# rodrigo-paganini/kalman-vae

Hardware: AMD Instinct MI355X
Metric: sequences/sec (ELBO training step, 32x32xT bouncing-ball) (higher is better)
Workload: dtype f32; 1 GPU; BASELINE configs[1] (configs[2] per-GPU shard): bouncing-ball 32x32, T=50, batch=256/GPU, dynamics=lstm K=3, z=4, u=4, a=2, full train step (fwd incl. sigmoid(x_logits) + loss incl. active-unit stats + bwd + clip + Adam); both the GPU leg and the cpu_baseline leg do this work; preset=c2, global_batch=256, seq_len=50, parallelism=dp1, capture=hipgraph, loss_finite=True, dist_backend=none

## Files before the change

### include/kvae_lgssm.h

```cpp
#ifndef KVAE_LGSSM_H
#define KVAE_LGSSM_H

#include <stdint.h>

#ifdef __cplusplus
extern "C" {
#endif

#define KVAE_MAX_DIM 16
#define KVAE_ABI_VERSION 11

typedef enum {
  KVAE_OK = 0,
  KVAE_ERR_DIMS = 1,
  KVAE_ERR_NULL = 2,
  KVAE_ERR_LAUNCH = 3,
  KVAE_ERR_ARG = 4
} kvae_status;

typedef struct {
  const float *ptr;
  int64_t sb, st;
} kvae_stack;

typedef struct {
  int32_t B, T, n, m, p;
  kvae_stack A;
  kvae_stack Bm;
  kvae_stack C;
  kvae_stack Q;
  const float *R;
  const float *mu0;
  int64_t mu0_sb;
// ... 125 lines not shown


int kvae_bce_frames_fwd(const float *logits, const float *x, float *frame_ll, int64_t frames, int32_t pixels, void *stream);
int kvae_bce_frames_bwd(const float *logits, const float *x, const float *g_frame, float *g_logits, int64_t frames,
                        int32_t pixels, void *stream);


#define KVAE_DEC_HEAD_SCRATCH_FLOATS 2304
int kvae_dec_head_fwd(const float *in, const float *W, const float *bias, float *logits, float *w_scratch, int64_t N,
                      int32_t Cin, int32_t side, void *stream);
int kvae_dec_head_bwd(const float *in, const float *W, const float *g_logits, float *g_in, float *w_partials,
                      float *b_partials, float *w_scratch, int64_t N, int32_t Cin, int32_t side, void *stream);
int kvae_enc_stem_fwd(const float *x, const float *W, const float *bias, float *out, uint32_t *relu_bits, int64_t N, int32_t Cout,
                      int32_t side, void *stream);
int kvae_enc_stem_bwd(const float *x, const float *out, const uint32_t *relu_bits, const float *g_out, float *w_partials,
                      float *b_partials, int64_t N, int32_t Cout, int32_t side, void *stream);
int64_t kvae_conv_edge_partial_rows(int64_t N);

int kvae_enc_mid_fwd(const float *in, const float *W, const float *bias, float *out, int64_t N, int32_t C, int32_t side,
                     void *stream);
int kvae_enc_mid_bwd(const float *in, const float *W, const float *out, const float *g_out, float *g_in,
                     float *w_partials, float *b_partials, int64_t N, int32_t C, int32_t side, void *stream);
int64_t kvae_enc_mid_partial_rows(int64_t N, int32_t side);

int kvae_dec_up_fwd(const float *x, const float *W, const float *bias, float *out, int64_t N, int32_t Cin, int32_t side,
                    void *stream);
int kvae_dec_up_bwd(const float *x, const float *W, const float *out, const float *g_out, float *g_x, float *w_partials,
                    float *b_partials, int64_t N, int32_t Cin, int32_t side, void *stream);
int64_t kvae_dec_up_partial_rows(int64_t N, int32_t side);
int32_t kvae_dec_up_set_workgroups(int32_t n);


int kvae_enc_head_fwd(const float *feat, const float *Wmu, const float *bmu, const float *Wvar, const float *bvar,
                      const float *eps, float *mu, float *var, float *a, int64_t N, int32_t F, int32_t A,
                      float noise_emission, void *stream);
int kvae_enc_head_bwd(const float *feat, const float *Wmu, const float *Wvar, const float *var, const float *eps,
                      const float *g_a, const float *g_mu, const float *g_var, float *g_feat, float *w_partials,
                      float *b_partials, int64_t N, int32_t F, int32_t A, float noise_emission, void *stream);
int kvae_dec_fc_fwd(const float *a, const float *W, const float *b, float *h, int64_t N, int32_t F, int32_t A, void *stream);
int kvae_dec_fc_bwd(const float *g_h, const float *a, const float *W, float *g_a, float *w_partials, float *b_partials,
                    int64_t N, int32_t F, int32_t A, void *stream);
int64_t kvae_head_partial_rows(void);
int kvae_latent_reg_fwd(const float *a, const float *mu, const float *var, float *reg, int64_t N, int32_t A, void *stream);
int kvae_latent_reg_bwd(const float *a, const float *mu, const float *var, const float *g, float *g_a, float *g_mu,
                        float *g_var, int64_t N, int32_t A, void *stream);

// ... 49 lines not shown
```

### kalman-vae_amd/csrc/kvae_vae.hip

```cpp
#include <hip/hip_runtime.h>

#include <stdint.h>
#include <stdio.h>
#include <stdlib.h>
#include <string.h>

#include "../../include/kvae_lgssm.h"

namespace kvae {}
using namespace kvae;

extern "C" int kvae_launch_status(const char *what);
static int launch_status(const char *what) { return kvae_launch_status(what); }

#include "vae_epilogue.h"

__device__ __forceinline__ void colsum_v4_body(const float *__restrict__ partials, float *__restrict__ out, int64_t rows, int64_t cols,
                                               unsigned block) {
  __shared__ float4 red[8][64];
  const int lane = threadIdx.x & 63, wv = threadIdx.x >> 6;
  const int64_t c = ((int64_t)block * 64 + lane) * 4;
  float4 s0 = make_float4(0.f, 0.f, 0.f, 0.f), s1 = s0, s2 = s0, s3 = s0;
  if (c < cols) {
    const float *p = partials + c;
// ... 399 lines not shown
  if (N < 1 || (N + 256 * 8) * EM_C * side * side * 4 >= EM_MAX_BYTES) return KVAE_ERR_ARG;
  if (C != EM_C || (side != 16 && side != 8)) return KVAE_ERR_DIMS;
  const dim3 grid((unsigned)enc_mid_grid(N, side));
  if (side == 16) k_enc_mid_fwd<16><<<grid, dim3(256), 0, (hipStream_t)stream>>>(in, W, bias, out, N);
  else k_enc_mid_fwd<8><<<grid, dim3(256), 0, (hipStream_t)stream>>>(in, W, bias, out, N);
  return launch_status("k_enc_mid_fwd");
}
int kvae_enc_mid_bwd(const float *in, const float *W, const float *out, const float *g_out, float *g_in,
                     float *w_partials, float *b_partials, int64_t N, int32_t C, int32_t side, void *stream) {
  if (!in || !W || !out || !g_out || !w_partials || !b_partials) return KVAE_ERR_NULL;
  if (N < 1 || (N + 256 * 8) * EM_C * side * side * 4 >= EM_MAX_BYTES) return KVAE_ERR_ARG;
  if (C != EM_C || (side != 16 && side != 8)) return KVAE_ERR_DIMS;
  const dim3 grid((unsigned)enc_mid_grid(N, side));
  if (g_in) {
    if (side == 16) k_enc_mid_bwd_data<16><<<grid, dim3(256), 0, (hipStream_t)stream>>>(W, out, g_out, g_in, N);
    else k_enc_mid_bwd_data<8><<<grid, dim3(256), 0, (hipStream_t)stream>>>(W, out, g_out, g_in, N);
    const int rc = launch_status("k_enc_mid_bwd_data");
    if (rc) return rc;
  }
  if (side == 16) k_enc_mid_wrw<16><<<grid, dim3(256), 0, (hipStream_t)stream>>>(in, out, g_out, w_partials, b_partials, N);
  else k_enc_mid_wrw<8><<<grid, dim3(256), 0, (hipStream_t)stream>>>(in, out, g_out, w_partials, b_partials, N);
  return launch_status("k_enc_mid_wrw");
}
}

#include "vae_conv_up_wino.h"
static bool dec_up_wino() {
  static const int env = getenv("KVAE_WINO") ? atoi(getenv("KVAE_WINO")) : 1;
  return env != 0;
}
static int g_dec_up_wgs = 0;
static inline int64_t dec_up_cap() {
  static const int env = getenv("KVAE_UP_WGS") ? atoi(getenv("KVAE_UP_WGS")) : 0;
  const int v = env >= 1 && env <= 256 ? env : __atomic_load_n(&g_dec_up_wgs, __ATOMIC_RELAXED);
  return v >= 1 && v <= 256 ? v : 256;
}
static inline int64_t dec_up_grid(int64_t N, int32_t side) {
  const int64_t fpi = side == 8 ? 2 : 8, iters = (N + fpi - 1) / fpi, cap = dec_up_cap();
  return iters < cap ? (iters < 1 ? 1 : iters) : cap;
}
extern "C" {
int64_t kvae_dec_up_partial_rows(int64_t N, int32_t side) { return dec_up_grid(N, side); }
int32_t kvae_dec_up_set_workgroups(int32_t n) {
  const int32_t prev = (int32_t)dec_up_cap();
  __atomic_store_n(&g_dec_up_wgs, n >= 1 && n <= 256 ? n : 0, __ATOMIC_RELAXED);
  return prev;
// ... 117 lines not shown
```

### kalman-vae_amd/csrc/vae_epilogue.h

```cpp
#pragma once
#include <stdint.h>

#include "lgssm_vm.h"

namespace kvae {

struct EpiShape { int64_t N; int C, H, W, r; };

KV_DEV int64_t epi_src(const EpiShape &s, int64_t o, int *ch) {
  const int OW = s.W * s.r, OH = s.H * s.r;
  const int ow = (int)(o % OW);
  const int64_t t1 = o / OW;
  const int oh = (int)(t1 % OH);
  const int64_t t2 = t1 / OH;
  const int c = (int)(t2 % s.C);
  const int64_t n = t2 / s.C;
  const int cc = c * s.r * s.r + (oh % s.r) * s.r + (ow % s.r);
  *ch = cc;
  return ((n * (s.C * s.r * s.r) + cc) * s.H + oh / s.r) * s.W + ow / s.r;
}

KV_DEV void epi_fwd_elem(const EpiShape &s, const float *in, const float *bias, float *out, int64_t o, int relu) {
  int ch;
  const int64_t i = epi_src(s, o, &ch);
  float v = in[i] + bias[ch];
  if (relu) v = v > 0.f ? v : 0.f;
  out[o] = v;
}

KV_DEV void epi_bwd_elem(const EpiShape &s, const float *g_out, const float *out, float *g_in, int64_t o, int relu) {
  int ch;
  const int64_t i = epi_src(s, o, &ch);
  float g = g_out[o];
  if (relu && !(out[o] > 0.f)) g = 0.f;
  g_in[i] = g;
}

}
```

### kalman-vae_amd/kvae/_native.py

```python
import ctypes as C
import os
from pathlib import Path

import torch

_HERE = Path(__file__).resolve().parent
LIB_PATH = _HERE / "lib" / "libkvae_lgssm.so"

KVAE_MAX_DIM = 16
KVAE_MAX_K = 16
LSTM_MAX_H, LSTM_MAX_I = 52, 16
ABI_VERSION = 11

_STATUS = {1: "KVAE_ERR_DIMS (n, m, p must be in [1,16]; B, T >= 1)", 2: "KVAE_ERR_NULL", 3: "KVAE_ERR_LAUNCH",
           4: "KVAE_ERR_ARG"}


class Stack(C.Structure):
    _fields_ = [("ptr", C.c_void_p), ("sb", C.c_int64), ("st", C.c_int64)]


class Problem(C.Structure):
    _fields_ = [("B", C.c_int32), ("T", C.c_int32), ("n", C.c_int32), ("m", C.c_int32), ("p", C.c_int32),
                ("A", Stack), ("Bm", Stack), ("C", Stack), ("Q", Stack),
                ("R", C.c_void_p), ("mu0", C.c_void_p), ("mu0_sb", C.c_int64),
                ("Sigma0", C.c_void_p), ("Sigma0_sb", C.c_int64),
                ("Y", C.c_void_p), ("U", C.c_void_p), ("mask", C.c_void_p)]


class States(C.Structure):
    _fields_ = [(k, C.c_void_p) for k in ("mus_filt", "Sigmas_filt", "mus_pred", "Sigmas_pred",
                                          "mus_smooth", "Sigmas_smooth", "aux")]


class WgradProblem(C.Structure):
    _fields_ = [("d", C.c_void_p), ("h", C.c_void_p), ("x", C.c_void_p), ("g_wh", C.c_void_p), ("g_wx", C.c_void_p),
                ("g_b", C.c_void_p), ("d_stride", C.c_int64), ("h_stride", C.c_int64), ("x_stride", C.c_int64), ("N", C.c_int64),
                ("R", C.c_int32), ("H", C.c_int32), ("I", C.c_int32), ("bias", C.c_int32), ("T", C.c_int32), ("shift", C.c_int32)]


class GenProblem(C.Structure):
    _fields_ = ([(k, C.c_int32) for k in ("B", "S", "H", "n", "m", "p", "K", "kind", "hidden")]
                + [(k, C.c_void_p) for k in ("A", "Bm", "C", "LQ", "LR", "mu", "L0", "U", "w_ih", "w_hh", "b_ih", "b_hh",
                                             "head_w", "head_b", "h0", "c0", "y0", "P", "s0", "eps0", "eps_z", "eps_a",
                                             "gumbel", "a_out", "z_out", "w_out")])


class InputGrads(C.Structure):
    _fields_ = [("gA", Stack), ("gB", Stack), ("gC", Stack), ("gQ", Stack),
                ("gY", C.c_void_p), ("gU", C.c_void_p), ("g_mu0", C.c_void_p), ("g_Sigma0", C.c_void_p)]


SYMBOLS = ("kvae_lgssm_filter_alpha_lstm", "kvae_lgssm_alpha_lstm_bwd", "kvae_lgssm_filter_fwd", "kvae_lgssm_rts_fwd", "kvae_lgssm_smooth_fwd", "kvae_lgssm_smooth_bwd",
           "kvae_lgssm_elbo", "kvae_mix_fwd", "kvae_mix_bwd", "kvae_mix_bwd_partials", "kvae_lstm_fwd",
           "kvae_lstm_bwd", "kvae_bias_shuffle_act_fwd", "kvae_bias_shuffle_act_bwd", "kvae_bias_partial_rows", "kvae_colsum", "kvae_colsum2", "kvae_clip_adam", "kvae_regime_fwd", "kvae_regime_bwd", "kvae_bigru_fwd", "kvae_bigru_bwd", "kvae_bce_frames_fwd", "kvae_bce_frames_bwd",
           "kvae_dec_head_fwd", "kvae_dec_head_bwd", "kvae_enc_stem_fwd", "kvae_enc_stem_bwd", "kvae_conv_edge_partial_rows",
           "kvae_enc_mid_fwd", "kvae_enc_mid_bwd", "kvae_enc_mid_partial_rows",
           "kvae_dec_up_fwd", "kvae_dec_up_bwd", "kvae_dec_up_partial_rows", "kvae_dec_up_set_workgroups",
           "kvae_enc_head_fwd", "kvae_enc_head_bwd", "kvae_dec_fc_fwd", "kvae_dec_fc_bwd", "kvae_head_partial_rows",
           "kvae_latent_reg_fwd", "kvae_latent_reg_bwd", "kvae_loss_head_fwd", "kvae_loss_head_bwd",
           "kvae_lgssm_emission_means", "kvae_lgssm_generate", "kvae_rnn_wgrad", "kvae_rnn_wgrad_ws_floats", "kvae_linear_fwd", "kvae_linear_bwd_input",
           "kvae_abi_version",
           "kvae_last_error", "kvae_build_info")


class LgssmLib:

    def __init__(self, path):
        self.path = str(path)
        self.dll = C.CDLL(self.path)
        missing = [s for s in SYMBOLS if not hasattr(self.dll, s)]
        if missing:
            raise OSError(f"{self.path} does not export {missing}")
        d = self.dll
        P, S, G, vp = C.POINTER(Problem), C.POINTER(States), C.POINTER(InputGrads), C.c_void_p
        for name in ("kvae_lgssm_filter_fwd", "kvae_lgssm_rts_fwd", "kvae_lgssm_smooth_fwd"):
            getattr(d, name).argtypes = [P, S, vp]
            getattr(d, name).restype = C.c_int
        d.kvae_lgssm_filter_alpha_lstm.argtypes = [P, S] + [vp] * 9 + [C.c_int32, C.c_int32] + [vp] * 7
        d.kvae_lgssm_filter_alpha_lstm.restype = C.c_int
# ... 24 lines not shown
        d.kvae_regime_bwd.argtypes = [vp] * 10 + [C.c_int32] * 3 + [C.c_float, vp, vp]
        d.kvae_regime_bwd.restype = C.c_int
        d.kvae_bigru_fwd.argtypes = [vp] * 7 + [C.c_int32] * 4 + [vp]
        d.kvae_bigru_fwd.restype = C.c_int
        d.kvae_bigru_bwd.argtypes = [vp] * 8 + [C.c_int32] * 4 + [vp]
        d.kvae_bigru_bwd.restype = C.c_int
        d.kvae_bce_frames_fwd.argtypes = [vp, vp, vp, C.c_int64, C.c_int32, vp]
        d.kvae_bce_frames_fwd.restype = C.c_int
        d.kvae_bce_frames_bwd.argtypes = [vp, vp, vp, vp, C.c_int64, C.c_int32, vp]
        d.kvae_bce_frames_bwd.restype = C.c_int
        d.kvae_dec_head_fwd.argtypes = [vp, vp, vp, vp, vp, C.c_int64, C.c_int32, C.c_int32, vp]
        d.kvae_dec_head_fwd.restype = C.c_int
        d.kvae_dec_head_bwd.argtypes = [vp] * 7 + [C.c_int64, C.c_int32, C.c_int32, vp]
        d.kvae_dec_head_bwd.restype = C.c_int
        d.kvae_enc_stem_fwd.argtypes = [vp, vp, vp, vp, vp, C.c_int64, C.c_int32, C.c_int32, vp]
        d.kvae_enc_stem_fwd.restype = C.c_int
        d.kvae_enc_stem_bwd.argtypes = [vp] * 6 + [C.c_int64, C.c_int32, C.c_int32, vp]
        d.kvae_enc_stem_bwd.restype = C.c_int
        d.kvae_enc_mid_fwd.argtypes = [vp, vp, vp, vp, C.c_int64, C.c_int32, C.c_int32, vp]
        d.kvae_enc_mid_fwd.restype = C.c_int
        d.kvae_enc_mid_bwd.argtypes = [vp] * 7 + [C.c_int64, C.c_int32, C.c_int32, vp]
        d.kvae_enc_mid_bwd.restype = C.c_int
        d.kvae_enc_mid_partial_rows.argtypes = [C.c_int64, C.c_int32]
        d.kvae_dec_up_fwd.argtypes = [vp, vp, vp, vp, C.c_int64, C.c_int32, C.c_int32, vp]
        d.kvae_dec_up_fwd.restype = C.c_int
        d.kvae_dec_up_bwd.argtypes = [vp] * 7 + [C.c_int64, C.c_int32, C.c_int32, vp]
        d.kvae_dec_up_bwd.restype = C.c_int
        d.kvae_dec_up_partial_rows.argtypes = [C.c_int64, C.c_int32]
        d.kvae_enc_head_fwd.argtypes = [vp] * 9 + [C.c_int64, C.c_int32, C.c_int32, C.c_float, vp]
        d.kvae_enc_head_fwd.restype = C.c_int
        d.kvae_enc_head_bwd.argtypes = [vp] * 11 + [C.c_int64, C.c_int32, C.c_int32, C.c_float, vp]
        d.kvae_enc_head_bwd.restype = C.c_int
        d.kvae_dec_fc_fwd.argtypes = [vp] * 4 + [C.c_int64, C.c_int32, C.c_int32, vp]
        d.kvae_dec_fc_fwd.restype = C.c_int
        d.kvae_dec_fc_bwd.argtypes = [vp] * 6 + [C.c_int64, C.c_int32, C.c_int32, vp]
        d.kvae_dec_fc_bwd.restype = C.c_int
        d.kvae_head_partial_rows.argtypes = []
        d.kvae_head_partial_rows.restype = C.c_int64
        d.kvae_latent_reg_fwd.argtypes = [vp] * 4 + [C.c_int64, C.c_int32, vp]
        d.kvae_latent_reg_fwd.restype = C.c_int
        d.kvae_latent_reg_bwd.argtypes = [vp] * 7 + [C.c_int64, C.c_int32, vp]
        d.kvae_latent_reg_bwd.restype = C.c_int
        d.kvae_loss_head_fwd.argtypes = [vp] * 5 + [C.c_float] * 3 + [vp, vp, vp, C.c_int64, vp]
        d.kvae_loss_head_fwd.restype = C.c_int
        d.kvae_loss_head_bwd.argtypes = [vp, vp, vp, vp, vp, vp, C.c_int64, vp]
        d.kvae_loss_head_bwd.restype = C.c_int
# ... 153 lines not shown
```

### kalman-vae_amd/kvae/vae/fused.py

```python
import torch

from .. import _native as N


colsum = N.colsum
colsum_pair = N.colsum_pair


def _chunks(n, size):
    return [(a, min(a + size, n)) for a in range(0, n, size)]


def _acc(total, part):
    return part if total is None else total + part


class BiasShuffleAct(torch.autograd.Function):

    @staticmethod
    def forward(ctx, x, bias, r, relu):
        x = x.contiguous()
        bias = bias.contiguous()
        Nb, Crr, H, W = x.shape
        C = Crr // (r * r)
# ... 120 lines not shown
            lib.check(N.timed(f"enc_mid_fwd_s{s}", x, lambda: lib.dll.kvae_enc_mid_fwd(
                N.ptr(x[a:b]), N.ptr(weight), N.ptr(bias), N.ptr(out[a:b]), b - a, Cc, s, N.stream_for(x))), "kvae_enc_mid_fwd")
        ctx.save_for_backward(x, weight, out)
        return out

    @staticmethod
    def backward(ctx, g):
        x, weight, out = ctx.saved_tensors
        g = g.contiguous()
        Nb, Cc, s, _ = x.shape
        lib = N.lib_for(x)
        g_x = torch.empty_like(x) if ctx.needs_input_grad[0] else None
        gw = gb = None
        for a, b in _chunks(Nb, EncoderMid.CHUNK):
            rows = lib.dll.kvae_enc_mid_partial_rows(b - a, s)
            wp = torch.empty(rows, weight.numel(), device=x.device, dtype=torch.float32)
            bp = torch.empty(rows, Cc, device=x.device, dtype=torch.float32)
            lib.check(lib.dll.kvae_enc_mid_bwd(N.ptr(x[a:b]), N.ptr(weight), N.ptr(out[a:b]), N.ptr(g[a:b]),
                                               N.ptr(g_x[a:b]) if g_x is not None else None, N.ptr(wp), N.ptr(bp), b - a, Cc, s,
                                               N.stream_for(x)), "kvae_enc_mid_bwd")
            cw, cb = colsum_pair(wp, bp)
            gw, gb = _acc(gw, cw), _acc(gb, cb)
        return g_x, gw.view_as(weight), gb


class DecoderUp(torch.autograd.Function):

    CHUNK = 16384

    @staticmethod
    def supported(x, conv):
        return (x.dim() == 4 and x.shape[1] == 32 and x.shape[2] == x.shape[3] and x.shape[2] in (8, 4)
                and tuple(conv.weight.shape) == (128, 32, 3, 3) and conv.stride == (1, 1) and conv.padding == (1, 1)
                and conv.dilation == (1, 1) and conv.groups == 1 and conv.bias is not None)

    @staticmethod
    def forward(ctx, x, weight, bias):
        x, weight, bias = x.contiguous(), weight.contiguous(), bias.contiguous()
        Nb, Cin, s, _ = x.shape
        out = torch.empty(Nb, 32, 2 * s, 2 * s, device=x.device, dtype=torch.float32)
        lib = N.lib_for(x)
        for a, b in _chunks(Nb, DecoderUp.CHUNK):
            lib.check(N.timed(f"dec_up_fwd_s{s}", x, lambda: lib.dll.kvae_dec_up_fwd(
                N.ptr(x[a:b]), N.ptr(weight), N.ptr(bias), N.ptr(out[a:b]), b - a, Cin, s, N.stream_for(x))), "kvae_dec_up_fwd")
        ctx.save_for_backward(x, weight, out)
        return out
# ... 185 lines not shown
```

### kalman-vae_amd/kvae/vae/vae.py

```python
import os
from typing import Tuple

import torch
import torch.nn as nn

from kvae import _native
from kvae.utils.config import KVAEConfig
from kvae.vae.fused import DecoderFc, DecoderHead, DecoderUp, EncoderHead, EncoderMid, EncoderStem, conv_block


def _conv_out(size, k, s, p):
    return (size + 2 * p - k) // s + 1


class Encoder(nn.Module):

    def __init__(self, config: KVAEConfig):
        super().__init__()
        self.config = config
        blocks, c_in, side = [], config.img_channels, config.img_size
        for c_out in config.encoder_channels:
            blocks += [nn.Conv2d(c_in, c_out, config.encoder_kernel_size, config.encoder_stride,
                                 config.encoder_padding), nn.ReLU()]
            side = _conv_out(side, config.encoder_kernel_size, config.encoder_stride, config.encoder_padding)
            c_in = c_out
        self.conv_layers = nn.Sequential(*blocks)
        self.flat_size = c_in * side * side
        self.fc_mu = nn.Linear(self.flat_size, config.a_dim)
        self.fc_var = nn.Sequential(nn.Linear(self.flat_size, config.a_dim), nn.Sigmoid())

    def features(self, x: torch.Tensor) -> torch.Tensor:
        if _native.fused_ok(x) and x.dtype == torch.float32:
            h = x
            for i, layer in enumerate(self.conv_layers):
                if isinstance(layer, nn.Conv2d):
                    if i == 0 and EncoderStem.supported(h, layer):
                        h = EncoderStem.apply(h, layer.weight, layer.bias)
                    elif EncoderMid.supported(h, layer):
                        h = EncoderMid.apply(h, layer.weight, layer.bias)
                    else:
                        h = conv_block(h, layer, r=1, relu=True)
            return h.flatten(1)
        return self.conv_layers(x).flatten(1)

    def heads(self, feat: torch.Tensor, eps=None):
        if _native.fused_ok(feat) and feat.dtype == torch.float32 and EncoderHead.supported(feat, self.fc_mu, self.fc_var[0]):
            return EncoderHead.apply(feat, self.fc_mu.weight, self.fc_mu.bias, self.fc_var[0].weight, self.fc_var[0].bias,
                                     eps, self.config.noise_emission)
        mu, var = self.fc_mu(feat), self.config.noise_emission * self.fc_var(feat)
        return (mu if eps is None else mu + eps * torch.sqrt(var + 1e-6)), mu, var

    def forward(self, x: torch.Tensor) -> Tuple[torch.Tensor, torch.Tensor]:
        _, mu, var = self.heads(self.features(x))
        return mu, var


class Decoder(nn.Module):
# ... 80 lines not shown
```

Before: 95460 sequences/s.

## Fuse encoder stem and mid conv layers into single kernels

Adds fused kernels that compute the first encoder conv (1->32, stride 2) together with the second conv (32->32, 16x16->8x8). The stem output stays in registers and LDS, interleaved with the MFMA work of the mid conv, so the intermediate activation is never written to or read back from global memory. Only packed ReLU bitmasks are stored. The backward pass recomputes stem activations from x to produce weight gradients for both layers in two kernels. This saves an activation round-trip and several launches, at the cost of very complex hand-scheduled kernels and recomputation work. The path is enabled by default through an env var and only applies when the batch fits in one chunk.

```diff
diff --git a/include/kvae_lgssm.h b/include/kvae_lgssm.h
--- a/include/kvae_lgssm.h
+++ b/include/kvae_lgssm.h
@@ -8,7 +8,7 @@
 #endif
 
 #define KVAE_MAX_DIM 16
-#define KVAE_ABI_VERSION 11
+#define KVAE_ABI_VERSION 12
 
 typedef enum {
   KVAE_OK = 0,
@@ -180,6 +180,13 @@
 int kvae_enc_mid_bwd(const float *in, const float *W, const float *out, const float *g_out, float *g_in,
                      float *w_partials, float *b_partials, int64_t N, int32_t C, int32_t side, void *stream);
 int64_t kvae_enc_mid_partial_rows(int64_t N, int32_t side);
+
+int kvae_enc_stem_mid_fwd(const float *x, const float *W0, const float *b0, const float *W1, const float *b1, float *out,
+                          uint32_t *relu_bits, int64_t N, void *stream);
+int kvae_enc_stem_mid_bwd(const float *x, const float *W0, const float *b0, const float *W1, const uint32_t *relu_bits,
+                          const float *out, const float *g_out, float *w0_partials, float *b0_partials, float *w1_partials,
+                          float *b1_partials, int64_t N, void *stream);
+int64_t kvae_enc_stem_mid_partial_rows(int64_t N);
 
 int kvae_dec_up_fwd(const float *x, const float *W, const float *bias, float *out, int64_t N, int32_t Cin, int32_t side,
                     void *stream);
diff --git a/kalman-vae_amd/csrc/kvae_vae.hip b/kalman-vae_amd/csrc/kvae_vae.hip
--- a/kalman-vae_amd/csrc/kvae_vae.hip
+++ b/kalman-vae_amd/csrc/kvae_vae.hip
@@ -445,6 +445,29 @@
   else k_enc_mid_wrw<8><<<grid, dim3(256), 0, (hipStream_t)stream>>>(in, out, g_out, w_partials, b_partials, N);
   return launch_status("k_enc_mid_wrw");
 }
+
+int64_t kvae_enc_stem_mid_partial_rows(int64_t N) { return enc_mid_grid(N, 16); }
+int kvae_enc_stem_mid_fwd(const float *x, const float *W0, const float *b0, const float *W1, const float *b1, float *out,
+                          uint32_t *relu_bits, int64_t N, void *stream) {
+  if (!x || !W0 || !b0 || !W1 || !b1 || !out || !relu_bits) return KVAE_ERR_NULL;
+  if (N < 1 || (N + 256 * 8) * EM_C * 16 * 16 * 4 >= EM_MAX_BYTES) return KVAE_ERR_ARG;
+  k_enc_stem_mid_fwd<<<dim3((unsigned)enc_mid_grid(N, 16)), dim3(256), 0, (hipStream_t)stream>>>(x, W0, b0, W1, b1, out, relu_bits, N);
+  return launch_status("k_enc_stem_mid_fwd");
+}
+int kvae_enc_stem_mid_bwd(const float *x, const float *W0, const float *b0, const float *W1, const uint32_t *relu_bits,
+                          const float *out, const float *g_out, float *w0_partials, float *b0_partials, float *w1_partials,
+                          float *b1_partials, int64_t N, void *stream) {
+  if (!x || !W0 || !b0 || !W1 || !relu_bits || !out || !g_out || !w0_partials || !b0_partials || !w1_partials || !b1_partials)
+    return KVAE_ERR_NULL;
+  if (N < 1 || (N + 256 * 8) * EM_C * 16 * 16 * 4 >= EM_MAX_BYTES) return KVAE_ERR_ARG;
+  const dim3 grid((unsigned)enc_mid_grid(N, 16));
+  k_enc_stem_mid_bwd<<<grid, dim3(256), 0, (hipStream_t)stream>>>(x, W1, relu_bits, out, g_out, w0_partials, b0_partials, N,
+                                                                  kvae_conv_edge_partial_rows(N));
+  const int rc = launch_status("k_enc_stem_mid_bwd");
+  if (rc) return rc;
+  k_enc_stem_mid_wrw<<<grid, dim3(256), 0, (hipStream_t)stream>>>(x, W0, b0, out, g_out, w1_partials, b1_partials, N);
+  return launch_status("k_enc_stem_mid_wrw");
+}
 }
 
 #include "vae_conv_up_wino.h"
diff --git a/kalman-vae_amd/csrc/vae_conv_stem_mid.h b/kalman-vae_amd/csrc/vae_conv_stem_mid.h
--- /dev/null
+++ b/kalman-vae_amd/csrc/vae_conv_stem_mid.h
@@ -0,0 +1,581 @@
+#pragma once
+#include <stdint.h>
+
+#include "../../include/kvae_lgssm.h"
+
+#if !defined(KVAE_HOSTSIM)
+#include "vae_conv_mid.h"
+
+namespace kvae {
+
+constexpr int ESM_TS = 35, ESM_TILE = 34 * ESM_TS;
+constexpr int ESM_OP = 258;
+typedef float esm_f4 __attribute__((ext_vector_type(4)));
+
+__device__ __forceinline__ void esm_fetch_frames(float4 (&xv)[2], __amdgpu_buffer_rsrc_t rx, int64_t i) {
+#pragma unroll
+  for (int u = 0; u < 2; ++u) xv[u] = em_ld4(rx, (uint32_t)(i * 2048 + (threadIdx.x + 256 * u) * 4) * 4u);
+}
+__device__ __forceinline__ void esm_put_frames(float *xt, const float4 (&xv)[2]) {
+#pragma unroll
+  for (int u = 0; u < 2; ++u) {
+    const int e = (threadIdx.x + 256 * u) * 4, f = e >> 10, h = (e >> 5) & 31, w = e & 31;
+    float *d = xt + f * ESM_TILE + (h + 1) * ESM_TS + w + 1;
+    d[0] = xv[u].x; d[1] = xv[u].y; d[2] = xv[u].z; d[3] = xv[u].w;
+  }
+}
+__device__ __forceinline__ void esm_window(float (&v)[9], const float *tile) {
+  const int oh = threadIdx.x >> 4, ow = threadIdx.x & 15;
+#pragma unroll
+  for (int ky = 0; ky < 3; ++ky)
+#pragma unroll
+    for (int kx = 0; kx < 3; ++kx) v[ky * 3 + kx] = tile[(2 * oh + ky) * ESM_TS + 2 * ow + kx];
+}
+constexpr int ESM_WS = 12;
+__device__ __forceinline__ void esm_load_stem_weights(float *w0l, const float *__restrict__ W0, const float *__restrict__ b0) {
+  for (int i = threadIdx.x; i < 32 * ESM_WS; i += 256) {
+    const int co = i / ESM_WS, k = i % ESM_WS;
+    w0l[i] = k == 0 ? b0[co] : (k < 10 ? W0[co * 9 + k - 1] : 0.f);
+  }
+}
+struct EsmW { float4 a, b, c; };
+__device__ __forceinline__ EsmW esm_wread(const float *w0l, int co) {
+  const float4 *p = reinterpret_cast<const float4 *>(w0l + co * ESM_WS);
+  return EsmW{p[0], p[1], p[2]};
+}
+#define ESM_OPAQUE(a) asm("" : "+v"(a))
+__device__ __forceinline__ float esm_chain(const float (&v)[9], const EsmW &w, int co, uint32_t &bits) {
+  const float wk[9] = {w.a.y, w.a.z, w.a.w, w.b.x, w.b.y, w.b.z, w.b.w, w.c.x, w.c.y};
+  float a = w.a.x;
+#pragma unroll
+  for (int k = 0; k < 9; ++k) {
+    ESM_OPAQUE(a);
+    a = fmaf(wk[k], v[k], a);
+  }
+  bits |= (a > 0.f ? 1u : 0u) << co;
+  return fmaxf(a, 0.f);
+}
+__device__ __forceinline__ void esm_stem2(const float (&v0)[9], const float (&v1)[9], const float *w0l, int co, float &o0, float &o1,
+                                          uint32_t &bits0, uint32_t &bits1) {
+  const float4 wa = reinterpret_cast<const float4 *>(w0l + co * ESM_WS)[0], wb = reinterpret_cast<const float4 *>(w0l + co * ESM_WS)[1],
+               wc = reinterpret_cast<const float4 *>(w0l + co * ESM_WS)[2];
+  const float w[9] = {wa.y, wa.z, wa.w, wb.x, wb.y, wb.z, wb.w, wc.x, wc.y};
+  float a0 = wa.x, a1 = wa.x;
+#pragma unroll
+  for (int k = 0; k < 9; ++k) {
+    ESM_OPAQUE(a0);
+    ESM_OPAQUE(a1);
+    a0 = fmaf(w[k], v0[k], a0);
+    a1 = fmaf(w[k], v1[k], a1);
+  }
+  bits0 |= (a0 > 0.f ? 1u : 0u) << co;
+  bits1 |= (a1 > 0.f ? 1u : 0u) << co;
+  o0 = fmaxf(a0, 0.f);
+  o1 = fmaxf(a1, 0.f);
+}
+
+__global__ __launch_bounds__(256) void k_enc_stem_mid_fwd(const float *__restrict__ x, const float *__restrict__ W0,
+                                                          const float *__restrict__ b0, const float *__restrict__ W,
+                                                          const float *__restrict__ bias, float *__restrict__ out,
+                                                          uint32_t *__restrict__ relu_bits, int64_t N) {
+  using D = EmDims<16>;
+  constexpr int S = 16;
+  __shared__ __attribute__((aligned(16))) float lds[32 * ESM_WS + EM_W + D::IT_IN + D::IT_OUT + 2 * ESM_TILE];
+  float *w0l = lds, *Wl = w0l + 32 * ESM_WS, *fr = Wl + EM_W, *ot = fr + D::IT_IN, *xt = ot + D::IT_OUT;
+  const int tid = threadIdx.x, lane = tid & 63, wv = tid >> 6, q = lane & 31, half = lane >> 5;
+  em_load_weights(Wl, W, true);
+  esm_load_stem_weights(w0l, W0, b0);
+  for (int i = tid; i < 2 * ESM_TILE; i += 256) xt[i] = 0.f;
+  const int64_t iters = (N + D::FPI - 1) / D::FPI, G = gridDim.x;
+  const int gp = 32 * wv + q, fl = gp / D::PF, pix = gp % D::PF, oh = pix / D::OS, ow = pix % D::OS;
+  const bool top = oh == 0, left = ow == 0;
+  const int bbase = fl * D::FRAME + half * D::PLANE + (2 * oh - 1) * S + (2 * ow - 1);
+  const int b_t = top ? EM_OOB : bbase, b_l = left ? EM_OOB : bbase, b_tl = (top || left) ? EM_OOB : bbase;
+  const int abase = half * 32 + q;
+  float bv[16];
+#pragma unroll
+  for (int r = 0; r < 16; ++r) bv[r] = bias[KV_ACC_ROW(r, half)];
+
+  const __amdgpu_buffer_rsrc_t rx = em_rsrc(x, N * 4096), rout = em_rsrc(out, N * EM_C * D::PF * 4),
+                               rb = em_rsrc(relu_bits, N * 1024);
+  auto store_bits = [&](int64_t i, int f, uint32_t bits) {
+    __builtin_amdgcn_raw_buffer_store_b32(bits, rb, (uint32_t)(i * 512 + f * 256 + tid) * 4u, 0, 0);
+  };
+  float pre[64], v0[9], v1[9];
+  float4 xv[2];
+  uint32_t bits0 = 0, bits1 = 0;
+  int64_t it = blockIdx.x;
+  esm_fetch_frames(xv, rx, it);
+  __syncthreads();
+  esm_put_frames(xt, xv);
+  esm_fetch_frames(xv, rx, it + G);
+  __syncthreads();
+  esm_window(v0, xt);
+  esm_window(v1, xt + ESM_TILE);
+#pragma unroll
+  for (int c = 0; c < 32; ++c) esm_stem2(v0, v1, w0l, c, pre[c], pre[32 + c], bits0, bits1);
+  store_bits(it, 0, bits0);
+  store_bits(it, 1, bits1);
+
+  uint32_t done_base = 0x80000000u;
+  auto flush1 = [&](int j) {
+    em_st4(rout, done_base + (uint32_t)(tid + 256 * j) * 16u, reinterpret_cast<const float4 *>(ot)[tid + 256 * j]);
+  };
+  for (; it < iters; it += G) {
+    __syncthreads();
+#pragma unroll
+    for (int j = 0; j < 64; ++j) fr[j * 256 + tid] = pre[j];
+    esm_put_frames(xt, xv);
+    __syncthreads();
+    em_f16 acc;
+#pragma unroll
+    for (int r = 0; r < 16; ++r) acc[r] = 0.f;
+    float av[36][4], bw[36][4];
+    auto rd = [&](int g) {
+#pragma unroll
+      for (int u = 0; u < 4; ++u) {
+        const int k = g * 4 + u, tap = k / 16, jj = k % 16, ky = tap / 3, kx = tap % 3;
+        av[g][u] = Wl[abase + (tap * 32 + 2 * jj) * 32];
+        bw[g][u] = fr[(ky == 0 ? (kx == 0 ? b_tl : b_t) : (kx == 0 ? b_l : bbase)) + ky * S + kx + 2 * jj * D::PLANE];
+      }
+    };
+    rd(0);
+    rd(1);
+    EsmW wq[37];
+#pragma unroll
+    for (int g = 0; g < 36; ++g) {
+      if (g + 2 < 36) rd(g + 2);
+      if (g < 4) flush1(g);
+      else if (g == 4) esm_fetch_frames(xv, rx, it + 2 * G);
+      if (g == 2) {
+        esm_window(v0, xt);
+        esm_window(v1, xt + ESM_TILE);
+        bits0 = bits1 = 0;
+      }
+      if (g >= 3 && g < 35) wq[g + 1] = esm_wread(w0l, g - 3);
+      __builtin_amdgcn_sched_barrier(0);
+      acc = KV_MFMA_F32(av[g][0], bw[g][0], acc);
+      __builtin_amdgcn_sched_barrier(0);
+      if (g >= 4) pre[g - 4] = esm_chain(v0, wq[g], g - 4, bits0);
+      __builtin_amdgcn_sched_barrier(0);
+      acc = KV_MFMA_F32(av[g][1], bw[g][1], acc);
+      __builtin_amdgcn_sched_barrier(0);
+      if (g >= 4) pre[32 + g - 4] = esm_chain(v1, wq[g], g - 4, bits1);
+      if (g == 35) {
+        store_bits(it + G, 0, bits0);
+        store_bits(it + G, 1, bits1);
+      }
+      __builtin_amdgcn_sched_barrier(0);
+      acc = KV_MFMA_F32(av[g][2], bw[g][2], acc);
+      acc = KV_MFMA_F32(av[g][3], bw[g][3], acc);
+      __builtin_amdgcn_sched_barrier(0);
+    }
+    __syncthreads();
+#pragma unroll
+    for (int r = 0; r < 16; ++r) ot[(fl * EM_C + KV_ACC_ROW(r, half)) * D::PF + pix] = fmaxf(acc[r] + bv[r], 0.f);
+    done_base = (uint32_t)(it * D::IT_OUT) * 4u;
+  }
+  __syncthreads();
+#pragma unroll
+  for (int j = 0; j < 4; ++j) flush1(j);
+}
+
+__global__ __launch_bounds__(256) void k_enc_stem_mid_bwd(const float *__restrict__ x, const float *__restrict__ W,
+                                                          const uint32_t *__restrict__ relu_bits, const float *__restrict__ out,
+                                                          const float *__restrict__ g_out, float *__restrict__ w_partials,
+                                                          float *__restrict__ b_partials, int64_t N, int64_t rows) {
+  using D = EmDims<16>;
+  constexpr int S = 16, OFR = EM_C * ESM_OP;
+  __shared__ float lds[EM_W + D::IT_OUT + 2 * OFR + 4 * ESM_TILE];
+  float *Wl = lds, *gm = lds + EM_W, *ot = gm + D::IT_OUT, *xt = ot + 2 * OFR;
+  const int tid = threadIdx.x, lane = tid & 63, wv = tid >> 6, q = lane & 31, half = lane >> 5;
+  em_load_weights(Wl, W, false);
+  for (int i = tid; i < 2 * OFR + 4 * ESM_TILE; i += 256) ot[i] = 0.f;
+  const int64_t iters = (N + D::FPI - 1) / D::FPI, total_out = N * EM_C * D::PF, G = gridDim.x;
+  const int cp = 32 * wv + q, fl = cp / D::PF, idx = cp % D::PF, a_ = idx / D::OS, b_ = idx % D::OS;
+  const bool bottom = a_ == D::OS - 1, right = b_ == D::OS - 1;
+  const int gbase = fl * EM_C * D::PF + half * D::PF + a_ * D::OS + b_;
+  const int g_b = bottom ? EM_OOB : gbase, g_r = right ? EM_OOB : gbase, g_br = (bottom || right) ? EM_OOB : gbase;
+  const int abase = half * 32 + q;
+  const int obase = fl * OFR + (2 * a_) * S + 2 * b_;
+  const int sj = lane & 15, sg = lane >> 4, stap = sj < 9 ? sj : 8;
+  const int tbo = (8 * wv) * ESM_TS + 2 * sg + (stap / 3) * ESM_TS + stap % 3;
+  const int gao = sj * ESM_OP + 64 * wv + sg;
+
+  const int rot = blockIdx.x & 15;
+  const __amdgpu_buffer_rsrc_t rg = em_rsrc(g_out, total_out * 4), ro = em_rsrc(out, total_out * 4),
+                               rx = em_rsrc(x, N * 4096), rb = em_rsrc(relu_bits, N * 1024);
+  float4 pg[4], po[4], xv[2];
+  uint32_t mn[2][2], mc[4];
+  int64_t it = blockIdx.x;
+  auto fetch1 = [&](int64_t i, int j) {
+    if (j < 8) {
+      const uint32_t e = (uint32_t)(i * D::IT_OUT + (tid + 256 * (((j & 3) + rot) & 3)) * 4) * 4u;
+      if (j < 4) pg[j] = em_ld4(rg, e);
+      else po[j - 4] = em_ld4(ro, e);
+    } else if (j < 10) {
+      xv[j - 8] = em_ld4(rx, (uint32_t)(i * 2048 + (tid + 256 * (j - 8)) * 4) * 4u);
+    } else {
+      const int ph = j - 10;
+      const auto w2 = __builtin_amdgcn_raw_buffer_load_b64(rb, (uint32_t)(i * 512 + fl * 256 + (2 * a_ + ph) * S + 2 * b_) * 4u, 0, 0);
+      mn[ph][0] = w2[0];
+      mn[ph][1] = w2[1];
+    }
+  };
+  esm_f4 sI[2][2], sO[2][2];
+#pragma unroll
+  for (int f = 0; f < 2; ++f)
+#pragma unroll
+    for (int hh = 0; hh < 2; ++hh) sI[f][hh] = sO[f][hh] = esm_f4{0.f, 0.f, 0.f, 0.f};
+  int img_par = 1;
+  float sa[16][2][2], sb[16][2];
+  auto srd = [&](const float *img, const float *tl, int h) {
+#pragma unroll
+    for (int u = 0; u < 2; ++u) {
+      const int f = h >> 3, s = 2 * (h & 7) + u;
+      const float xb = tl[f * ESM_TILE + tbo + 2 * (s >> 2) * ESM_TS + 8 * (s & 3)];
+      sb[h][u] = sj == 9 ? 1.0f : xb;
+      sa[h][u][0] = img[f * OFR + gao + 4 * s];
+      sa[h][u][1] = img[f * OFR + gao + 16 * ESM_OP + 4 * s];
+    }
+  };
+  auto smfma = [&](int h) {
+    const int f = h >> 3;
+#pragma unroll
+    for (int u = 0; u < 2; ++u) {
+      sI[f][0] = __builtin_amdgcn_mfma_f32_16x16x4f32(sa[h][u][0], sb[h][u], sI[f][0], 0, 0, 0);
+      sI[f][1] = __builtin_amdgcn_mfma_f32_16x16x4f32(sa[h][u][1], sb[h][u], sI[f][1], 0, 0, 0);
+    }
+  };
+  float *xcur = xt, *xprev = xt + 2 * ESM_TILE;
+#pragma unroll
+  for (int j = 0; j < 12; ++j) fetch1(it, j);
+  for (; it < iters; it += G) {
+    __syncthreads();
+#pragma unroll
+    for (int j = 0; j < 4; ++j)
+      reinterpret_cast<float4 *>(gm)[tid + 256 * ((j + rot) & 3)] =
+          make_float4(po[j].x > 0.f ? pg[j].x : 0.f, po[j].y > 0.f ? pg[j].y : 0.f, po[j].z > 0.f ? pg[j].z : 0.f,
+                      po[j].w > 0.f ? pg[j].w : 0.f);
+    esm_put_frames(xcur, xv);
+#pragma unroll
+    for (int ph = 0; ph < 2; ++ph) {
+      mc[2 * ph] = mn[ph][0];
+      mc[2 * ph + 1] = mn[ph][1];
+    }
+    __syncthreads();
+    constexpr int E_CLS[9] = {3, 3, 3, 3, 1, 1, 2, 2, 0};
+    constexpr int E_KY[9] = {0, 0, 2, 2, 1, 1, 0, 2, 1};
+    constexpr int E_KX[9] = {0, 2, 0, 2, 0, 2, 1, 1, 1};
+    float av[36][4], bw[36][4];
+    auto rd = [&](int g) {
+#pragma unroll
+      for (int u = 0; u < 4; ++u) {
+        const int en = g / 4, jj = (g % 4) * 4 + u, ph = E_CLS[en] >> 1, pw = E_CLS[en] & 1;
+        const int dy = (ph == 1 && E_KY[en] == 0) ? 1 : 0, dx = (pw == 1 && E_KX[en] == 0) ? 1 : 0;
+        av[g][u] = Wl[abase + ((E_KY[en] * 3 + E_KX[en]) * 32 + 2 * jj) * 32];
+        bw[g][u] = gm[(dy ? (dx ? g_br : g_b) : (dx ? g_r : gbase)) + 2 * jj * D::PF + dy * D::OS + dx];
+      }
+    };
+    rd(0);
+    rd(1);
+    srd(ot, xprev, 0);
+    em_f16 acc;
+#pragma unroll
+    for (int g = 0; g < 36; ++g) {
+      const int en = g / 4, cls = E_CLS[en], ph = cls >> 1, pw = cls & 1;
+      if (g % 4 == 0 && (en == 0 || E_CLS[en - 1] != cls)) {
+#pragma unroll
+        for (int r = 0; r < 16; ++r) acc[r] = 0.f;
+      }
+      if (g + 2 < 36) rd(g + 2);
+      if (g + 1 < 16) srd(ot, xprev, g + 1);
+      if (g < 12) fetch1(it + G, g);
+      __builtin_amdgcn_sched_barrier(0);
+#pragma unroll
+      for (int u = 0; u < 4; ++u) acc = KV_MFMA_F32(av[g][u], bw[g][u], acc);
+      if (g < 16) smfma(g);
+      __builtin_amdgcn_sched_barrier(0);
+      if (g % 4 == 3 && (en == 8 || E_CLS[en + 1] != cls)) {
+        if (g == 15) __syncthreads();
+        const uint32_t m = mc[2 * ph + pw] >> (4 * half);
+#pragma unroll
+        for (int r = 0; r < 16; ++r)
+          ot[obase + KV_ACC_ROW(r, half) * ESM_OP + ph * S + pw] = (m >> KV_ACC_ROW(r, 0)) & 1u ? acc[r] : 0.f;
+      }
+    }
+    float *t = xcur;
+    xcur = xprev;
+    xprev = t;
+#pragma unroll
+    for (int f = 0; f < 2; ++f)
+#pragma unroll
+      for (int hh = 0; hh < 2; ++hh) {
+        const esm_f4 s = sI[f][hh];
+        sI[f][hh] = sO[f][hh];
+        sO[f][hh] = s;
+      }
+    img_par ^= 1;
+  }
+  __syncthreads();
+#pragma unroll
+  for (int h = 0; h < 16; ++h) {
+    srd(ot, xprev, h);
+    smfma(h);
+  }
+  float *red = gm;
+#pragma unroll
+  for (int set = 0; set < 2; ++set)
+#pragma unroll
+    for (int f = 0; f < 2; ++f) {
+      const int par = set == 0 ? img_par : img_par ^ 1;
+      const int64_t row = 2 * (int64_t)blockIdx.x + f + 512 * par;
+      __syncthreads();
+#pragma unroll
+      for (int r = 0; r < 4; ++r) {
+        red[(wv * 32 + 4 * sg + r) * 16 + sj] = set == 0 ? sI[f][0][r] : sO[f][0][r];
+        red[(wv * 32 + 16 + 4 * sg + r) * 16 + sj] = set == 0 ? sI[f][1][r] : sO[f][1][r];
+      }
+      __syncthreads();
+      if (row < rows) {
+        for (int o = tid; o < EM_C * 10; o += 256) {
+          const int c = o / 10, k = o - c * 10;
+          const float s = (red[c * 16 + k] + red[(32 + c) * 16 + k]) + (red[(64 + c) * 16 + k] + red[(96 + c) * 16 + k]);
+          if (k < 9) w_partials[row * (EM_C * 9) + c * 9 + k] = s;
+          else b_partials[row * EM_C + c] = s;
+        }
+      }
+    }
+}
+
+__global__ __launch_bounds__(256) void k_enc_stem_mid_wrw(const float *__restrict__ x, const float *__restrict__ W0,
+                                                          const float *__restrict__ b0, const float *__restrict__ out,
+                                                          const float *__restrict__ g_out, float *__restrict__ w_partials,
+                                                          float *__restrict__ b_partials, int64_t N) {
+  using D = EmDims<16>;
+  constexpr int S = 16, CSP = D::PLANE + 1, GSP = D::PF + 1;
+  constexpr int XS = D::FPI * EM_C * CSP;
+  __shared__ __attribute__((aligned(16))) float lds[32 * ESM_WS + D::FPI * EM_C * GSP + 2 * XS + 2 * ESM_TILE];
+  float *w0l = lds, *gm = lds + 32 * ESM_WS, *xcur = gm + D::FPI * EM_C * GSP, *xnxt = xcur + XS, *xt = xnxt + XS;
+  const int tid = threadIdx.x, lane = tid & 63, wv = tid >> 6, q = lane & 31, half = lane >> 5;
+  esm_load_stem_weights(w0l, W0, b0);
+  for (int i = tid; i < 2 * ESM_TILE; i += 256) xt[i] = 0.f;
+  const int64_t iters = (N + D::FPI - 1) / D::FPI, total_out = N * EM_C * D::PF, G = gridDim.x;
+  const int wframe = wv >> 1, wpix0 = 32 * (wv & 1);
+  const int oh0 = wpix0 / D::OS;
+  const int abase = wframe * EM_C * GSP + q * GSP + wpix0 + half;
+  const int bbase = wframe * EM_C * CSP + q * CSP + (2 * oh0 - 1) * S - 1 + 2 * half;
+  const bool wtop = oh0 == 0, wleft = half == 0;
+  const int x_t = wtop ? EM_OOB : bbase, x_l = wleft ? EM_OOB : bbase, x_tl = (wtop || wleft) ? EM_OOB : bbase;
+
+  em_f16 acc[9];
+#pragma unroll
+  for (int t = 0; t < 9; ++t)
+#pragma unroll
+    for (int r = 0; r < 16; ++r) acc[t][r] = 0.f;
+  float bsum = 0.f;
+
+  const int rot = blockIdx.x & 15;
+  const __amdgpu_buffer_rsrc_t rx = em_rsrc(x, N * 4096), rg = em_rsrc(g_out, total_out * 4), ro = em_rsrc(out, total_out * 4);
+  float4 pg[4], po[4], xv[2];
+  float v0[9], v1[9];
+  uint32_t bits0 = 0, bits1 = 0;
+  int64_t it = blockIdx.x;
+  auto fetch1 = [&](int64_t i, int j) {
+    const uint32_t e = (uint32_t)(i * D::IT_OUT + (tid + 256 * (((j & 3) + rot) & 3)) * 4) * 4u;
+    if (j < 4) pg[j] = em_ld4(rg, e);
+    else po[j - 4] = em_ld4(ro, e);
+  };
+#pragma unroll
+  for (int j = 0; j < 8; ++j) fetch1(it, j);
+  esm_fetch_frames(xv, rx, it);
+  __syncthreads();
+  esm_put_frames(xt, xv);
+  esm_fetch_frames(xv, rx, it + G);
+  __syncthreads();
+  esm_window(v0, xt);
+  esm_window(v1, xt + ESM_TILE);
+#pragma unroll
+  for (int c = 0; c < 32; ++c) {
+    float o0, o1;
+    esm_stem2(v0, v1, w0l, c, o0, o1, bits0, bits1);
+    xnxt[c * CSP + tid] = o0;
+    xnxt[(32 + c) * CSP + tid] = o1;
+  }
+  for (; it < iters; it += G) {
+    __syncthreads();
+    {
+      float *t = xcur;
+      xcur = xnxt;
+      xnxt = t;
+    }
+    esm_put_frames(xt, xv);
+#pragma unroll
+    for (int j = 0; j < 4; ++j) {
+      const int e = (tid + 256 * ((j + rot) & 3)) * 4, f = e / (EM_C * D::PF), c = (e / D::PF) % EM_C, p = e % D::PF;
+      float *d = gm + (f * EM_C + c) * GSP + p;
+      d[0] = po[j].x > 0.f ? pg[j].x : 0.f; d[1] = po[j].y > 0.f ? pg[j].y : 0.f;
+      d[2] = po[j].z > 0.f ? pg[j].z : 0.f; d[3] = po[j].w > 0.f ? pg[j].w : 0.f;
+    }
+    __syncthreads();
+    float av[16], bw[16][9];
+    auto rd = [&](int i) {
+      const int p = 2 * i, ohr = p / D::OS, owr = p % D::OS;
+      av[i] = gm[abase + p];
+#pragma unroll
+      for (int tap = 0; tap < 9; ++tap) {
+        const bool zt = tap / 3 == 0 && ohr == 0, zl = tap % 3 == 0 && owr == 0;
+        bw[i][tap] = xcur[(zt ? (zl ? x_tl : x_t) : (zl ? x_l : bbase)) + (2 * ohr + tap / 3) * S + 2 * owr + tap % 3];
+      }
+    };
+    EsmW wq[16][2];
+    rd(0);
+    esm_window(v0, xt);
+    esm_window(v1, xt + ESM_TILE);
+#pragma unroll
+    for (int i = 0; i < 16; ++i) {
+      if (i + 1 < 16) rd(i + 1);
+      wq[i][0] = esm_wread(w0l, 2 * i);
+      wq[i][1] = esm_wread(w0l, 2 * i + 1);
+      if (i < 8) fetch1(it + G, i);
+      else if (i == 8) esm_fetch_frames(xv, rx, it + 2 * G);
+      __builtin_amdgcn_sched_barrier(0);
+      bsum += av[i];
+#pragma unroll
+      for (int tap = 0; tap < 9; ++tap) {
+        acc[tap] = KV_MFMA_F32(av[i], bw[i][tap], acc[tap]);
+        if (tap < 8 && (tap & 1) == 0) {
+          __builtin_amdgcn_sched_barrier(0);
+          const int u = tap >> 2, c = 2 * i + u;
+          if ((tap & 2) == 0) xnxt[c * CSP + tid] = esm_chain(v0, wq[i][u], c, bits0);
+          else xnxt[(32 + c) * CSP + tid] = esm_chain(v1, wq[i][u], c, bits1);
+          __builtin_amdgcn_sched_barrier(0);
+        }
+      }
+      __builtin_amdgcn_sched_barrier(0);
+    }
+  }
+  float *red = lds, *redb = lds + EM_W;
+  for (int w = 0; w < 4; ++w) {
+    __syncthreads();
+    if (wv == w) {
+#pragma unroll
+      for (int tap = 0; tap < 9; ++tap)
+#pragma unroll
+        for (int r = 0; r < 16; ++r) {
+          float *d = red + (KV_ACC_ROW(r, half) * EM_C + q) * 9 + tap;
+          *d = w == 0 ? acc[tap][r] : *d + acc[tap][r];
+        }
+      float *db = redb + half * EM_C + q;
+      *db = w == 0 ? bsum : *db + bsum;
+    }
+  }
+  __syncthreads();
+  for (int i = tid; i < EM_W; i += 256) w_partials[(int64_t)blockIdx.x * EM_W + i] = red[i];
+  if (tid < EM_C) b_partials[(int64_t)blockIdx.x * EM_C + tid] = redb[tid] + redb[EM_C + tid];
+}
+
+}
+
+#else
+#include <math.h>
+#include <string.h>
+
+extern "C" {
+static void esm_stem_frame_sim(const float *x, const float *W0, const float *b0, float *h, uint32_t *bits) {
+  for (int p = 0; p < 256; ++p) bits[p] = 0;
+  for (int co = 0; co < 32; ++co)
+    for (int oh = 0; oh < 16; ++oh)
+      for (int ow = 0; ow < 16; ++ow) {
+        float acc = b0[co];
+        for (int ky = 0; ky < 3; ++ky)
+          for (int kx = 0; kx < 3; ++kx) {
+            const int y = 2 * oh + ky - 1, xx = 2 * ow + kx - 1;
+            const float v = (y < 0 || y >= 32 || xx < 0 || xx >= 32) ? 0.f : x[y * 32 + xx];
+            acc = fmaf(W0[co * 9 + ky * 3 + kx], v, acc);
+          }
+        h[(co * 16 + oh) * 16 + ow] = acc > 0.f ? acc : 0.f;
+        bits[oh * 16 + ow] |= (acc > 0.f ? 1u : 0u) << co;
+      }
+}
+int64_t kvae_enc_stem_mid_partial_rows(int64_t N) {
+  const int64_t iters = (N + 1) / 2;
+  return iters < 256 ? (iters < 1 ? 1 : iters) : 256;
+}
+int kvae_enc_stem_mid_fwd(const float *x, const float *W0, const float *b0, const float *W1, const float *b1, float *out,
+                          uint32_t *relu_bits, int64_t N, void *) {
+  if (!x || !W0 || !b0 || !W1 || !b1 || !out || !relu_bits) return KVAE_ERR_NULL;
+  if (N < 1) return KVAE_ERR_ARG;
+  float h[32 * 256];
+  for (int64_t n = 0; n < N; ++n) {
+    esm_stem_frame_sim(x + n * 1024, W0, b0, h, relu_bits + n * 256);
+    for (int co = 0; co < 32; ++co)
+      for (int oh = 0; oh < 8; ++oh)
+        for (int ow = 0; ow < 8; ++ow) {
+          float acc = b1[co];
+          for (int ci = 0; ci < 32; ++ci)
+            for (int ky = 0; ky < 3; ++ky)
+              for (int kx = 0; kx < 3; ++kx) {
+                const int y = 2 * oh + ky - 1, xx = 2 * ow + kx - 1;
+                if (y < 0 || y >= 16 || xx < 0 || xx >= 16) continue;
+                acc += W1[((co * 32 + ci) * 3 + ky) * 3 + kx] * h[(ci * 16 + y) * 16 + xx];
+              }
+          out[((n * 32 + co) * 8 + oh) * 8 + ow] = acc > 0.f ? acc : 0.f;
+        }
+  }
+  return KVAE_OK;
+}
+int kvae_enc_stem_mid_bwd(const float *x, const float *W0, const float *b0, const float *W1, const uint32_t *relu_bits,
+                          const float *out, const float *g_out, float *w0_partials, float *b0_partials, float *w1_partials,
+                          float *b1_partials, int64_t N, void *) {
+  if (!x || !W0 || !b0 || !W1 || !relu_bits || !out || !g_out || !w0_partials || !b0_partials || !w1_partials || !b1_partials)
+    return KVAE_ERR_NULL;
+  if (N < 1) return KVAE_ERR_ARG;
+  const int64_t rows0 = kvae_conv_edge_partial_rows(N), rows = kvae_enc_stem_mid_partial_rows(N);
+  memset(w0_partials, 0, sizeof(float) * rows0 * 288);
+  memset(b0_partials, 0, sizeof(float) * rows0 * 32);
+  memset(w1_partials, 0, sizeof(float) * rows * 9216);
+  memset(b1_partials, 0, sizeof(float) * rows * 32);
+  float h[32 * 256], gh[32 * 256];
+  uint32_t bits[256];
+  for (int64_t n = 0; n < N; ++n) {
+    float *wp0 = w0_partials + (n % rows0) * 288, *bp0 = b0_partials + (n % rows0) * 32;
+    float *wp1 = w1_partials + (n % rows) * 9216, *bp1 = b1_partials + (n % rows) * 32;
+    const float *xf = x + n * 1024;
+    esm_stem_frame_sim(xf, W0, b0, h, bits);
+    memset(gh, 0, sizeof(gh));
+    for (int co = 0; co < 32; ++co)
+      for (int oh = 0; oh < 8; ++oh)
+        for (int ow = 0; ow < 8; ++ow) {
+          const int64_t oi = ((n * 32 + co) * 8 + oh) * 8 + ow;
+          if (!(out[oi] > 0.f)) continue;
+          const float g = g_out[oi];
+          bp1[co] += g;
+          for (int ci = 0; ci < 32; ++ci)
+            for (int ky = 0; ky < 3; ++ky)
+              for (int kx = 0; kx < 3; ++kx) {
+                const int y = 2 * oh + ky - 1, xx = 2 * ow + kx - 1;
+                if (y < 0 || y >= 16 || xx < 0 || xx >= 16) continue;
+                const int wi = ((co * 32 + ci) * 3 + ky) * 3 + kx, hi = (ci * 16 + y) * 16 + xx;
+                wp1[wi] += g * h[hi];
+                gh[hi] += g * W1[wi];
+              }
+        }
+    for (int co = 0; co < 32; ++co)
+      for (int p = 0; p < 256; ++p) {
+        if (!((relu_bits[n * 256 + p] >> co) & 1u)) continue;
+        const float g = gh[co * 256 + p];
+        const int oh = p >> 4, ow = p & 15;
+        bp0[co] += g;
+        for (int ky = 0; ky < 3; ++ky)
+          for (int kx = 0; kx < 3; ++kx) {
+            const int y = 2 * oh + ky - 1, xx = 2 * ow + kx - 1;
+            if (y < 0 || y >= 32 || xx < 0 || xx >= 32) continue;
+            wp0[co * 9 + ky * 3 + kx] += g * xf[y * 32 + xx];
+          }
+      }
+  }
+  return KVAE_OK;
+}
+}
+#endif
diff --git a/kalman-vae_amd/csrc/vae_epilogue.h b/kalman-vae_amd/csrc/vae_epilogue.h
--- a/kalman-vae_amd/csrc/vae_epilogue.h
+++ b/kalman-vae_amd/csrc/vae_epilogue.h
@@ -37,3 +37,5 @@
 }
 
 }
+
+#include "vae_conv_stem_mid.h"
diff --git a/kalman-vae_amd/kvae/_native.py b/kalman-vae_amd/kvae/_native.py
--- a/kalman-vae_amd/kvae/_native.py
+++ b/kalman-vae_amd/kvae/_native.py
@@ -10,7 +10,7 @@
 KVAE_MAX_DIM = 16
 KVAE_MAX_K = 16
 LSTM_MAX_H, LSTM_MAX_I = 52, 16
-ABI_VERSION = 11
+ABI_VERSION = 12
 
 _STATUS = {1: "KVAE_ERR_DIMS (n, m, p must be in [1,16]; B, T >= 1)", 2: "KVAE_ERR_NULL", 3: "KVAE_ERR_LAUNCH",
            4: "KVAE_ERR_ARG"}
@@ -56,6 +56,7 @@
            "kvae_lstm_bwd", "kvae_bias_shuffle_act_fwd", "kvae_bias_shuffle_act_bwd", "kvae_bias_partial_rows", "kvae_colsum", "kvae_colsum2", "kvae_clip_adam", "kvae_regime_fwd", "kvae_regime_bwd", "kvae_bigru_fwd", "kvae_bigru_bwd", "kvae_bce_frames_fwd", "kvae_bce_frames_bwd",
            "kvae_dec_head_fwd", "kvae_dec_head_bwd", "kvae_enc_stem_fwd", "kvae_enc_stem_bwd", "kvae_conv_edge_partial_rows",
            "kvae_enc_mid_fwd", "kvae_enc_mid_bwd", "kvae_enc_mid_partial_rows",
+           "kvae_enc_stem_mid_fwd", "kvae_enc_stem_mid_bwd", "kvae_enc_stem_mid_partial_rows",
            "kvae_dec_up_fwd", "kvae_dec_up_bwd", "kvae_dec_up_partial_rows", "kvae_dec_up_set_workgroups",
            "kvae_enc_head_fwd", "kvae_enc_head_bwd", "kvae_dec_fc_fwd", "kvae_dec_fc_bwd", "kvae_head_partial_rows",
            "kvae_latent_reg_fwd", "kvae_latent_reg_bwd", "kvae_loss_head_fwd", "kvae_loss_head_bwd",
@@ -126,6 +127,12 @@
         d.kvae_enc_mid_bwd.argtypes = [vp] * 7 + [C.c_int64, C.c_int32, C.c_int32, vp]
         d.kvae_enc_mid_bwd.restype = C.c_int
         d.kvae_enc_mid_partial_rows.argtypes = [C.c_int64, C.c_int32]
+        d.kvae_enc_stem_mid_fwd.argtypes = [vp] * 7 + [C.c_int64, vp]
+        d.kvae_enc_stem_mid_fwd.restype = C.c_int
+        d.kvae_enc_stem_mid_bwd.argtypes = [vp] * 11 + [C.c_int64, vp]
+        d.kvae_enc_stem_mid_bwd.restype = C.c_int
+        d.kvae_enc_stem_mid_partial_rows.argtypes = [C.c_int64]
+        d.kvae_enc_stem_mid_partial_rows.restype = C.c_int64
         d.kvae_dec_up_fwd.argtypes = [vp, vp, vp, vp, C.c_int64, C.c_int32, C.c_int32, vp]
         d.kvae_dec_up_fwd.restype = C.c_int
         d.kvae_dec_up_bwd.argtypes = [vp] * 7 + [C.c_int64, C.c_int32, C.c_int32, vp]
diff --git a/kalman-vae_amd/kvae/vae/fused.py b/kalman-vae_amd/kvae/vae/fused.py
--- a/kalman-vae_amd/kvae/vae/fused.py
+++ b/kalman-vae_amd/kvae/vae/fused.py
@@ -166,6 +166,51 @@
             cw, cb = colsum_pair(wp, bp)
             gw, gb = _acc(gw, cw), _acc(gb, cb)
         return g_x, gw.view_as(weight), gb
+
+
+class EncoderStemMid(torch.autograd.Function):
+
+    CHUNK = EncoderMid.CHUNK
+    _STEM_OUT = torch.empty((1, 32, 16, 16), device="meta")
+
+    @staticmethod
+    def supported(x, stem, mid):
+        return EncoderStem.supported(x, stem) and EncoderMid.supported(EncoderStemMid._STEM_OUT, mid)
+
+    @staticmethod
+    def forward(ctx, x, W0, b0, W1, b1):
+        x, W0, b0, W1, b1 = (t.contiguous() for t in (x, W0, b0, W1, b1))
+        Nb = x.shape[0]
+        out = torch.empty(Nb, 32, 8, 8, device=x.device, dtype=torch.float32)
+        bits = torch.empty(Nb, 256, device=x.device, dtype=torch.int32)
+        lib = N.lib_for(x)
+        for a, b in _chunks(Nb, EncoderStemMid.CHUNK):
+            lib.check(lib.dll.kvae_enc_stem_mid_fwd(N.ptr(x[a:b]), N.ptr(W0), N.ptr(b0), N.ptr(W1), N.ptr(b1), N.ptr(out[a:b]),
+                                                    N.ptr(bits[a:b]), b - a, N.stream_for(x)), "kvae_enc_stem_mid_fwd")
+        ctx.save_for_backward(x, bits, W0, b0, W1, out)
+        return out
+
+    @staticmethod
+    def backward(ctx, g):
+        x, bits, W0, b0, W1, out = ctx.saved_tensors
+        g = g.contiguous()
+        Nb = x.shape[0]
+        lib = N.lib_for(x)
+        gw0 = gb0 = gw1 = gb1 = None
+        for a, b in _chunks(Nb, EncoderStemMid.CHUNK):
+            rows = lib.dll.kvae_enc_stem_mid_partial_rows(b - a)
+            rows0 = lib.dll.kvae_conv_edge_partial_rows(b - a)
+            wp0 = torch.empty(rows0, W0.numel(), device=x.device, dtype=torch.float32)
+            bp0 = torch.empty(rows0, 32, device=x.device, dtype=torch.float32)
+            wp1 = torch.empty(rows, W1.numel(), device=x.device, dtype=torch.float32)
+            bp1 = torch.empty(rows, 32, device=x.device, dtype=torch.float32)
+            lib.check(lib.dll.kvae_enc_stem_mid_bwd(N.ptr(x[a:b]), N.ptr(W0), N.ptr(b0), N.ptr(W1), N.ptr(bits[a:b]), N.ptr(out[a:b]),
+                                                    N.ptr(g[a:b]), N.ptr(wp0), N.ptr(bp0), N.ptr(wp1), N.ptr(bp1), b - a,
+                                                    N.stream_for(x)), "kvae_enc_stem_mid_bwd")
+            cw1, cb1 = colsum_pair(wp1, bp1)
+            cw0, cb0 = colsum_pair(wp0, bp0)
+            gw1, gb1, gw0, gb0 = _acc(gw1, cw1), _acc(gb1, cb1), _acc(gw0, cw0), _acc(gb0, cb0)
+        return None, gw0.view_as(W0), gb0, gw1.view_as(W1), gb1
 
 
 class DecoderUp(torch.autograd.Function):
diff --git a/kalman-vae_amd/kvae/vae/vae.py b/kalman-vae_amd/kvae/vae/vae.py
--- a/kalman-vae_amd/kvae/vae/vae.py
+++ b/kalman-vae_amd/kvae/vae/vae.py
@@ -6,7 +6,8 @@
 
 from kvae import _native
 from kvae.utils.config import KVAEConfig
-from kvae.vae.fused import DecoderFc, DecoderHead, DecoderUp, EncoderHead, EncoderMid, EncoderStem, conv_block
+from kvae.vae.fused import (DecoderFc, DecoderHead, DecoderUp, EncoderHead, EncoderMid, EncoderStem, EncoderStemMid,
+                            conv_block)
 
 
 def _conv_out(size, k, s, p):
@@ -32,7 +33,15 @@
     def features(self, x: torch.Tensor) -> torch.Tensor:
         if _native.fused_ok(x) and x.dtype == torch.float32:
             h = x
-            for i, layer in enumerate(self.conv_layers):
+            layers = list(self.conv_layers)
+            start = 0
+            if (os.environ.get("KVAE_ENC_FUSE", "1") != "0" and len(layers) >= 4 and isinstance(layers[2], nn.Conv2d)
+                    and h.shape[0] <= EncoderStemMid.CHUNK and EncoderStemMid.supported(h, layers[0], layers[2])):
+                h = EncoderStemMid.apply(h, layers[0].weight, layers[0].bias, layers[2].weight, layers[2].bias)
+                start = 4
+            for i, layer in enumerate(layers):
+                if i < start:
+                    continue
                 if isinstance(layer, nn.Conv2d):
                     if i == 0 and EncoderStem.supported(h, layer):
                         h = EncoderStem.apply(h, layer.weight, layer.bias)
```

Result: faster. 97170 sequences/s, median of 6 (+1.8%).
